# naver/dust3r

Hardware: NVIDIA H100
Metric: image-pairs/sec (512x384, ViT-L/B+DPT) (higher is better)
Workload: dtype bf16

## Files before the change

### dust3r_b200/csrc/attention_wgmma.cu

```cuda
#include "d3r_common.cuh"
#include "sm90_ptx.cuh"
#include "elementwise.h"
#include "prof.h"
#include "pdl.cuh"

namespace d3r {
namespace attn {

namespace wg {

constexpr int BQ = 128, BK = 128, D = 64;
constexpr int kThreads = 384;
constexpr int kTileBytes = 128 * 64 * 2;
constexpr int kPBytes = 2 * 64 * 128 * 2;
template <bool P_SMEM>
struct Smem {
  static constexpr int kP = P_SMEM ? 2 * kPBytes : 0;
  static constexpr int kBytes = kTileBytes  + 2 * kTileBytes  + 2 * kTileBytes  + kP + 128  + 1024;
  static_assert(kBytes <= 227 * 1024, "shared memory of one CTA");
};

template <bool P_SMEM>
__global__ void __launch_bounds__(kThreads, 1)
attention_kernel(const __grid_constant__ CUtensorMap tmap_q, const __grid_constant__ CUtensorMap tmap_k,
                 const __grid_constant__ CUtensorMap tmap_v, __nv_bfloat16* __restrict__ out, long long ldo, int Nq, int Nk,
                 int heads, int total_tiles, float scale_log2) {
  extern __shared__ uint8_t smem_raw[];
  uint8_t* smem = reinterpret_cast<uint8_t*>((reinterpret_cast<uintptr_t>(smem_raw) + 1023) & ~uintptr_t(1023));
  uint8_t* s_q = smem;
  uint8_t* s_k = s_q + kTileBytes;
  uint8_t* s_v = s_k + 2 * kTileBytes;
  uint8_t* s_p = s_v + 2 * kTileBytes;
  uint64_t* bars = reinterpret_cast<uint64_t*>(s_p + Smem<P_SMEM>::kP);
  uint64_t* q_full = bars + 0;
  uint64_t* q_empty = bars + 1;
  uint64_t* k_full = bars + 2;
  uint64_t* k_empty = bars + 4;
  uint64_t* v_full = bars + 6;
  uint64_t* v_empty = bars + 8;

  const int warp = threadIdx.x >> 5, lane = threadIdx.x & 31;
  const int nq_tiles = (Nq + BQ - 1) / BQ;
  const int nblk = (Nk + BK - 1) / BK;
  auto tile_coords = [&](int t, int& q0, int& h, int& b) {
    q0 = (t % nq_tiles) * BQ;
    h = (t / nq_tiles) % heads;
    b = t / (nq_tiles * heads);
  };

  if (threadIdx.x == 0) {
    ptx::prefetch_tmap(&tmap_q);
    ptx::prefetch_tmap(&tmap_k);
    ptx::prefetch_tmap(&tmap_v);
    ptx::mbar_init(ptx::smem_u32(q_full), 1);
    ptx::mbar_init(ptx::smem_u32(q_empty), 8);
    for (int s = 0; s < 2; ++s) {
      ptx::mbar_init(ptx::smem_u32(&k_full[s]), 1);
      ptx::mbar_init(ptx::smem_u32(&k_empty[s]), 8);
      ptx::mbar_init(ptx::smem_u32(&v_full[s]), 1);
      ptx::mbar_init(ptx::smem_u32(&v_empty[s]), 8);
    }
    ptx::fence_barrier_init();
  }
  __syncthreads();
  pdl::sync_with_predecessor();

  if (warp < 4) {
    ptx::setmaxnreg_dec<24>();
    if (warp == 0 && ptx::elect_one()) {
      uint32_t g = 0, it = 0;
      for (int t = blockIdx.x; t < total_tiles; t += gridDim.x, ++it) {
        int q0, h, b;
        tile_coords(t, q0, h, b);
        ptx::mbar_wait(ptx::smem_u32(q_empty), (it & 1) ^ 1);
        ptx::mbar_arrive_expect_tx(ptx::smem_u32(q_full), kTileBytes);
        ptx::tma_load_3d(ptx::smem_u32(s_q), &tmap_q, ptx::smem_u32(q_full), h * D, q0, b);
        for (int j = 0; j < nblk; ++j, ++g) {
          const int st = g & 1;
          const uint32_t ph = (g >> 1) & 1;
          ptx::mbar_wait(ptx::smem_u32(&k_empty[st]), ph ^ 1);
          ptx::mbar_arrive_expect_tx(ptx::smem_u32(&k_full[st]), kTileBytes);
          ptx::tma_load_3d(ptx::smem_u32(s_k + st * kTileBytes), &tmap_k, ptx::smem_u32(&k_full[st]), h * D, j * BK, b);
          ptx::mbar_wait(ptx::smem_u32(&v_empty[st]), ph ^ 1);
          ptx::mbar_arrive_expect_tx(ptx::smem_u32(&v_full[st]), kTileBytes);
          ptx::tma_load_3d(ptx::smem_u32(s_v + st * kTileBytes), &tmap_v, ptx::smem_u32(&v_full[st]), h * D, j * BK, b);
        }
      }
    }
  } else {
    ptx::setmaxnreg_inc<240>();
    const int cw = (threadIdx.x >> 7) - 1;
    const int wq = warp & 3, q = lane & 3;
    uint8_t* s_pw = s_p + cw * kPBytes;
    uint32_t g = 0, it = 0;
    for (int t = blockIdx.x; t < total_tiles; t += gridDim.x, ++it) {
      int q0, h, b;
      tile_coords(t, q0, h, b);
      float m_run[2] = {-INFINITY, -INFINITY}, l_run[2] = {0.f, 0.f};
      float o[32];
#pragma unroll
      for (int i = 0; i < 32; ++i) o[i] = 0.f;
      ptx::mbar_wait(ptx::smem_u32(q_full), it & 1);
      const uint64_t dq = ptx::desc_kmajor_sw128(ptx::smem_u32(s_q + cw * 64 * 128));
      for (int j = 0; j < nblk; ++j, ++g) {
        const int st = g & 1;
        const uint32_t ph = (g >> 1) & 1;
        float s[64];
        ptx::mbar_wait(ptx::smem_u32(&k_full[st]), ph);
        const uint64_t dk = ptx::desc_kmajor_sw128(ptx::smem_u32(s_k + st * kTileBytes));
        ptx::wgmma_fence();
#pragma unroll
        for (int k = 0; k < D / 16; ++k) ptx::wgmma_m64n128k16_ss(s, dq + uint64_t(2 * k), dk + uint64_t(2 * k), k ? 1u : 0u);
        ptx::wgmma_commit();
        ptx::wgmma_wait<0>();
        ptx::reg_fence(s);
        if (lane == 0) {
          ptx::mbar_arrive(ptx::smem_u32(&k_empty[st]));
          if (j == nblk - 1) ptx::mbar_arrive(ptx::smem_u32(q_empty));
        }
        const int nvalid = Nk - j * BK;
        if (nvalid < BK) {
#pragma unroll
          for (int n = 0; n < 16; ++n)
#pragma unroll
            for (int e = 0; e < 2; ++e)
              if (8 * n + 2 * q + e >= nvalid) { s[4 * n + e] = -INFINITY; s[4 * n + 2 + e] = -INFINITY; }
        }
        float ms[2];
#pragma unroll
        for (int hh = 0; hh < 2; ++hh) {
          float mx = -INFINITY;
#pragma unroll
          for (int n = 0; n < 16; ++n) mx = fmaxf(mx, fmaxf(s[4 * n + 2 * hh], s[4 * n + 2 * hh + 1]));
          mx = fmaxf(mx, __shfl_xor_sync(0xffffffffu, mx, 1));
          mx = fmaxf(mx, __shfl_xor_sync(0xffffffffu, mx, 2));
          const float m_new = fmaxf(m_run[hh], mx);
          const float corr = ptx::ex2_approx((m_run[hh] - m_new) * scale_log2);
          m_run[hh] = m_new;
          l_run[hh] *= corr;
#pragma unroll
          for (int n = 0; n < 8; ++n) { o[4 * n + 2 * hh] *= corr; o[4 * n + 2 * hh + 1] *= corr; }
          ms[hh] = m_new * scale_log2;
        }
        uint32_t pk[32];
#pragma unroll
        for (int n = 0; n < 16; ++n)
#pragma unroll
          for (int hh = 0; hh < 2; ++hh) {
            const float p0 = ptx::ex2_approx(fmaf(s[4 * n + 2 * hh], scale_log2, -ms[hh]));
            const float p1 = ptx::ex2_approx(fmaf(s[4 * n + 2 * hh + 1], scale_log2, -ms[hh]));
            l_run[hh] += p0 + p1;
            pk[2 * n + hh] = pack_bf16x2(p0, p1);
          }
        ptx::mbar_wait(ptx::smem_u32(&v_full[st]), ph);
        const uint32_t sv = ptx::smem_u32(s_v + st * kTileBytes);
        if constexpr (P_SMEM) {
#pragma unroll
          for (int n = 0; n < 16; ++n)
#pragma unroll
            for (int hh = 0; hh < 2; ++hh) {
              const int r = wq * 16 + (lane >> 2) + 8 * hh;
              *reinterpret_cast<uint32_t*>(s_pw + (n >> 3) * (64 * 128) + r * 128 + (((n & 7) ^ (r & 7)) << 4) + 4 * q) = pk[2 * n + hh];
            }
          ptx::fence_proxy_async();
          asm volatile("bar.sync %0, 128;" ::"r"(1 + cw) : "memory");
          const uint32_t sp = ptx::smem_u32(s_pw);
          ptx::wgmma_fence();
#pragma unroll
          for (int kk = 0; kk < BK / 16; ++kk)
            ptx::wgmma_m64n64k16_ss_tb(o, ptx::desc_kmajor_sw128(sp + (kk >> 2) * (64 * 128)) + uint64_t(2 * (kk & 3)),
                                       ptx::desc_mnmajor_sw128(sv + kk * 16 * 128), 1u);
        } else {
          ptx::wgmma_fence();
#pragma unroll
          for (int kk = 0; kk < BK / 16; ++kk) ptx::wgmma_m64n64k16_rs_tb(o, pk + 4 * kk, ptx::desc_mnmajor_sw128(sv + kk * 16 * 128), 1u);
        }
        ptx::wgmma_commit();
        ptx::wgmma_wait<0>();
        ptx::reg_fence(o);
        if constexpr (P_SMEM) asm volatile("bar.sync %0, 128;" ::"r"(1 + cw) : "memory");
        if (lane == 0) ptx::mbar_arrive(ptx::smem_u32(&v_empty[st]));
      }
#pragma unroll
      for (int hh = 0; hh < 2; ++hh) {
        float l = l_run[hh];
        l += __shfl_xor_sync(0xffffffffu, l, 1);
        l += __shfl_xor_sync(0xffffffffu, l, 2);
        const float inv = 1.f / l;
        const int qrow = q0 + cw * 64 + wq * 16 + (lane >> 2) + 8 * hh;
        if (qrow < Nq) {
          __nv_bfloat16* orow = out + ((long long)b * Nq + qrow) * ldo + h * D + 2 * q;
#pragma unroll
          for (int n = 0; n < 8; ++n)
            *reinterpret_cast<uint32_t*>(orow + 8 * n) = pack_bf16x2(o[4 * n + 2 * hh] * inv, o[4 * n + 2 * hh + 1] * inv);
        }
      }
    }
  }
}

}

template <bool P_SMEM>
static int launch_attention(const CUtensorMap& mq, const CUtensorMap& mk, const CUtensorMap& mv, void* out, long long ldo, int B, int heads,
                            int Nq, int Nk, float scale, cudaStream_t st) {
  static unsigned long long attr_devices = 0;
  if (first_launch_on_this_device(attr_devices))
    D3R_CUDA(cudaFuncSetAttribute(wg::attention_kernel<P_SMEM>, cudaFuncAttributeMaxDynamicSharedMemorySize, wg::Smem<P_SMEM>::kBytes));
  const int total_tiles = ((Nq + wg::BQ - 1) / wg::BQ) * heads * B;
  const int slots = num_sms();
  const int rounds = (total_tiles + slots - 1) / slots;
  const int grid = (total_tiles + rounds - 1) / rounds;
  prof::Scope scope(P_SMEM ? "attention_wgmma_psmem" : "attention_wgmma", st, 4.0 * double(B) * heads * double(Nq) * double(Nk) * 64.0);
  D3R_CUDA(pdl::launch(wg::attention_kernel<P_SMEM>, dim3(grid), dim3(wg::kThreads), size_t(wg::Smem<P_SMEM>::kBytes), st, mq, mk, mv,
                       (__nv_bfloat16*)out, ldo, Nq, Nk, heads, total_tiles, scale * 1.4426950408889634f));
  D3R_LAUNCH_CHECK();
  return D3R_OK;
}

static int make_map(CUtensorMap* m, const void* base, long long ld, int cols, int N, int B, int box_rows) {
  const cuuint64_t dims[3] = {(cuuint64_t)cols, (cuuint64_t)N, (cuuint64_t)B};
  const cuuint64_t str[2] = {(cuuint64_t)ld * 2, (cuuint64_t)N * ld * 2};
  const cuuint32_t box[3] = {64, (cuuint32_t)box_rows, 1};
  return encode_tensor_map(m, base, 3, dims, str, box, "attention");
}

static int g_impl = 3;

int attention_hd64(const void* q, long long ldq, const void* k, long long ldk, const void* v, long long ldv, void* out,
                   long long ldo, int B, int heads, int Nq, int Nk, float scale, cudaStream_t st) {
  D3R_CHECK_ARG(q && k && v && out && B > 0 && heads > 0 && Nq > 0 && Nk > 0, "attention: bad arguments");
  D3R_CHECK_ARG(ldq % 8 == 0 && ldk % 8 == 0 && ldv % 8 == 0 && ldo % 8 == 0, "attention: row strides must be multiples of 8");
  D3R_CHECK_ARG(((uintptr_t)q & 15) == 0 && ((uintptr_t)k & 15) == 0 && ((uintptr_t)v & 15) == 0 && ((uintptr_t)out & 15) == 0,
                "attention: pointers must be 16-byte aligned");
  CUtensorMap mq, mk, mv;
  int rc;
  if ((rc = make_map(&mq, q, ldq, heads * 64, Nq, B, wg::BQ))) return rc;
  if ((rc = make_map(&mk, k, ldk, heads * 64, Nk, B, wg::BK))) return rc;
  if ((rc = make_map(&mv, v, ldv, heads * 64, Nk, B, wg::BK))) return rc;
  if (g_impl == 2) return launch_attention<true>(mq, mk, mv, out, ldo, B, heads, Nq, Nk, scale, st);
  return launch_attention<false>(mq, mk, mv, out, ldo, B, heads, Nq, Nk, scale, st);
}

}
}

extern "C" void d3r_set_attention_impl(int32_t impl) { d3r::attn::g_impl = (impl == 2) ? 2 : 3; }

extern "C" int d3r_attention_hd64(const void* q, int64_t ldq, const void* k, int64_t ldk, const void* v, int64_t ldv, void* out,
                                  int64_t ldo, int32_t B, int32_t heads, int32_t Nq, int32_t Nk, float scale, void* stream) {
  return d3r::attn::attention_hd64(q, ldq, k, ldk, v, ldv, out, ldo, B, heads, Nq, Nk, scale, (cudaStream_t)stream);
}
```

Before: 234.3.

## Pipeline QK^T and PV WGMMAs across key blocks with three consumer warpgroups

```diff
diff --git a/dust3r_b200/csrc/attention_wgmma.cu b/dust3r_b200/csrc/attention_wgmma.cu
--- a/dust3r_b200/csrc/attention_wgmma.cu
+++ b/dust3r_b200/csrc/attention_wgmma.cu
@@ -9,56 +9,135 @@
 
 namespace wg {
 
-constexpr int BQ = 128, BK = 128, D = 64;
-constexpr int kThreads = 384;
+constexpr int BK = 128, D = 64;
 constexpr int kTileBytes = 128 * 64 * 2;
 constexpr int kPBytes = 2 * 64 * 128 * 2;
-template <bool P_SMEM>
-struct Smem {
-  static constexpr int kP = P_SMEM ? 2 * kPBytes : 0;
-  static constexpr int kBytes = kTileBytes  + 2 * kTileBytes  + 2 * kTileBytes  + kP + 128  + 1024;
-  static_assert(kBytes <= 227 * 1024, "shared memory of one CTA");
+constexpr int kSerialReg = 1, kSmemP = 2, kPipelined = 3;
+template <int IMPL>
+struct Cfg {
+  static constexpr bool kPSmem = IMPL == kSmemP;
+  static constexpr bool kPipe = IMPL == kPipelined;
+  static constexpr int kConsumers = kPipe ? 3 : 2;
+  static constexpr int BQ = 64 * kConsumers;
+  static constexpr int kThreads = 128 * (1 + kConsumers);
+  static constexpr int kConsumerRegs = kConsumers == 3 ? 160 : 240;
+  static_assert(128 * (24 + kConsumers * kConsumerRegs) <= 65536, "register file of one SM");
+  static constexpr int kStages = 2;
+  static constexpr int kP = kPSmem ? 2 * kPBytes : 0;
+  static constexpr int kSmemBytes =
+      BQ * 128  + kStages * kTileBytes  + kStages * kTileBytes  + kP + 128  + 1024;
+  static_assert(kSmemBytes <= 227 * 1024, "shared memory of one CTA");
+  static_assert(4 * kStages + 2 <= 16, "barriers fit their 128 bytes");
 };
 
-template <bool P_SMEM>
-__global__ void __launch_bounds__(kThreads, 1)
+
+__device__ __forceinline__ void mask_keys(float (&s)[64], int nvalid, int q) {
+  if (nvalid < BK) {
+#pragma unroll
+    for (int n = 0; n < 16; ++n)
+#pragma unroll
+      for (int e = 0; e < 2; ++e)
+        if (8 * n + 2 * q + e >= nvalid) { s[4 * n + e] = -INFINITY; s[4 * n + 2 + e] = -INFINITY; }
+  }
+}
+
+__device__ __forceinline__ void softmax_max(const float (&s)[64], float (&m_run)[2], float (&l_run)[2], float (&corr)[2],
+                                            float (&ms)[2], float scale_log2) {
+#pragma unroll
+  for (int hh = 0; hh < 2; ++hh) {
+    float mx = -INFINITY;
+#pragma unroll
+    for (int n = 0; n < 16; ++n) mx = fmaxf(mx, fmaxf(s[4 * n + 2 * hh], s[4 * n + 2 * hh + 1]));
+    mx = fmaxf(mx, __shfl_xor_sync(0xffffffffu, mx, 1));
+    mx = fmaxf(mx, __shfl_xor_sync(0xffffffffu, mx, 2));
+    const float m_new = fmaxf(m_run[hh], mx);
+    corr[hh] = ptx::ex2_approx((m_run[hh] - m_new) * scale_log2);
+    m_run[hh] = m_new;
+    l_run[hh] *= corr[hh];
+    ms[hh] = m_new * scale_log2;
+  }
+}
+
+__device__ __forceinline__ void rescale_o(float (&o)[32], const float (&corr)[2]) {
+#pragma unroll
+  for (int hh = 0; hh < 2; ++hh)
+#pragma unroll
+    for (int n = 0; n < 8; ++n) { o[4 * n + 2 * hh] *= corr[hh]; o[4 * n + 2 * hh + 1] *= corr[hh]; }
+}
+
+__device__ __forceinline__ void softmax_exp(float (&s)[64], const float (&ms)[2], float (&l_run)[2], float scale_log2) {
+#pragma unroll
+  for (int n = 0; n < 16; ++n)
+#pragma unroll
+    for (int hh = 0; hh < 2; ++hh) {
+      const float p0 = ptx::ex2_approx(fmaf(s[4 * n + 2 * hh], scale_log2, -ms[hh]));
+      const float p1 = ptx::ex2_approx(fmaf(s[4 * n + 2 * hh + 1], scale_log2, -ms[hh]));
+      l_run[hh] += p0 + p1;
+      s[4 * n + 2 * hh] = p0;
+      s[4 * n + 2 * hh + 1] = p1;
+    }
+}
+
+__device__ __forceinline__ void pack_p(const float (&p)[64], uint32_t (&pk)[32]) {
+#pragma unroll
+  for (int n = 0; n < 16; ++n)
+#pragma unroll
+    for (int hh = 0; hh < 2; ++hh) pk[2 * n + hh] = pack_bf16x2(p[4 * n + 2 * hh], p[4 * n + 2 * hh + 1]);
+}
+
+__device__ __forceinline__ void issue_s(float (&s)[64], uint64_t dq, uint64_t dk) {
+#pragma unroll
+  for (int k = 0; k < D / 16; ++k) ptx::wgmma_m64n128k16_ss(s, dq + uint64_t(2 * k), dk + uint64_t(2 * k), k ? 1u : 0u);
+}
+
+__device__ __forceinline__ void issue_pv_reg(float (&o)[32], const uint32_t (&pk)[32], uint32_t sv) {
+#pragma unroll
+  for (int kk = 0; kk < BK / 16; ++kk) ptx::wgmma_m64n64k16_rs_tb(o, pk + 4 * kk, ptx::desc_mnmajor_sw128(sv + kk * 16 * 128), 1u);
+}
+
+template <int IMPL>
+__global__ void __launch_bounds__(Cfg<IMPL>::kThreads, 1)
 attention_kernel(const __grid_constant__ CUtensorMap tmap_q, const __grid_constant__ CUtensorMap tmap_k,
                  const __grid_constant__ CUtensorMap tmap_v, __nv_bfloat16* __restrict__ out, long long ldo, int Nq, int Nk,
                  int heads, int total_tiles, float scale_log2) {
+  using C = Cfg<IMPL>;
+  constexpr int S = C::kStages;
   extern __shared__ uint8_t smem_raw[];
   uint8_t* smem = reinterpret_cast<uint8_t*>((reinterpret_cast<uintptr_t>(smem_raw) + 1023) & ~uintptr_t(1023));
   uint8_t* s_q = smem;
-  uint8_t* s_k = s_q + kTileBytes;
-  uint8_t* s_v = s_k + 2 * kTileBytes;
-  uint8_t* s_p = s_v + 2 * kTileBytes;
-  uint64_t* bars = reinterpret_cast<uint64_t*>(s_p + Smem<P_SMEM>::kP);
+  uint8_t* s_k = s_q + C::BQ * 128;
+  uint8_t* s_v = s_k + S * kTileBytes;
+  uint8_t* s_p = s_v + S * kTileBytes;
+  uint64_t* bars = reinterpret_cast<uint64_t*>(s_p + C::kP);
   uint64_t* q_full = bars + 0;
   uint64_t* q_empty = bars + 1;
   uint64_t* k_full = bars + 2;
-  uint64_t* k_empty = bars + 4;
-  uint64_t* v_full = bars + 6;
-  uint64_t* v_empty = bars + 8;
+  uint64_t* k_empty = bars + 2 + S;
+  uint64_t* v_full = bars + 2 + 2 * S;
+  uint64_t* v_empty = bars + 2 + 3 * S;
 
   const int warp = threadIdx.x >> 5, lane = threadIdx.x & 31;
-  const int nq_tiles = (Nq + BQ - 1) / BQ;
+  const int nq_tiles = (Nq + C::BQ - 1) / C::BQ;
   const int nblk = (Nk + BK - 1) / BK;
   auto tile_coords = [&](int t, int& q0, int& h, int& b) {
-    q0 = (t % nq_tiles) * BQ;
+    q0 = (t % nq_tiles) * C::BQ;
     h = (t / nq_tiles) % heads;
     b = t / (nq_tiles * heads);
   };
+  auto stage = [](uint32_t g) { return int(g % S); };
+  auto phase = [](uint32_t g) { return (g / S) & 1u; };
 
   if (threadIdx.x == 0) {
     ptx::prefetch_tmap(&tmap_q);
     ptx::prefetch_tmap(&tmap_k);
     ptx::prefetch_tmap(&tmap_v);
     ptx::mbar_init(ptx::smem_u32(q_full), 1);
-    ptx::mbar_init(ptx::smem_u32(q_empty), 8);
-    for (int s = 0; s < 2; ++s) {
+    ptx::mbar_init(ptx::smem_u32(q_empty), 4 * C::kConsumers);
+    for (int s = 0; s < S; ++s) {
       ptx::mbar_init(ptx::smem_u32(&k_full[s]), 1);
-      ptx::mbar_init(ptx::smem_u32(&k_empty[s]), 8);
+      ptx::mbar_init(ptx::smem_u32(&k_empty[s]), 4 * C::kConsumers);
       ptx::mbar_init(ptx::smem_u32(&v_full[s]), 1);
-      ptx::mbar_init(ptx::smem_u32(&v_empty[s]), 8);
+      ptx::mbar_init(ptx::smem_u32(&v_empty[s]), 4 * C::kConsumers);
     }
     ptx::fence_barrier_init();
   }
@@ -73,11 +152,11 @@
         int q0, h, b;
         tile_coords(t, q0, h, b);
         ptx::mbar_wait(ptx::smem_u32(q_empty), (it & 1) ^ 1);
-        ptx::mbar_arrive_expect_tx(ptx::smem_u32(q_full), kTileBytes);
+        ptx::mbar_arrive_expect_tx(ptx::smem_u32(q_full), C::BQ * 128);
         ptx::tma_load_3d(ptx::smem_u32(s_q), &tmap_q, ptx::smem_u32(q_full), h * D, q0, b);
         for (int j = 0; j < nblk; ++j, ++g) {
-          const int st = g & 1;
-          const uint32_t ph = (g >> 1) & 1;
+          const int st = stage(g);
+          const uint32_t ph = phase(g);
           ptx::mbar_wait(ptx::smem_u32(&k_empty[st]), ph ^ 1);
           ptx::mbar_arrive_expect_tx(ptx::smem_u32(&k_full[st]), kTileBytes);
           ptx::tma_load_3d(ptx::smem_u32(s_k + st * kTileBytes), &tmap_k, ptx::smem_u32(&k_full[st]), h * D, j * BK, b);
@@ -88,10 +167,15 @@
       }
     }
   } else {
-    ptx::setmaxnreg_inc<240>();
+    ptx::setmaxnreg_inc<C::kConsumerRegs>();
     const int cw = (threadIdx.x >> 7) - 1;
     const int wq = warp & 3, q = lane & 3;
     uint8_t* s_pw = s_p + cw * kPBytes;
+    auto k_smem = [&](uint32_t g) { return ptx::smem_u32(s_k + stage(g) * kTileBytes); };
+    auto v_smem = [&](uint32_t g) { return ptx::smem_u32(s_v + stage(g) * kTileBytes); };
+    auto release = [&](uint64_t* bar) {
+      if (lane == 0) ptx::mbar_arrive(ptx::smem_u32(bar));
+    };
     uint32_t g = 0, it = 0;
     for (int t = blockIdx.x; t < total_tiles; t += gridDim.x, ++it) {
       int q0, h, b;
@@ -102,84 +186,99 @@
       for (int i = 0; i < 32; ++i) o[i] = 0.f;
       ptx::mbar_wait(ptx::smem_u32(q_full), it & 1);
       const uint64_t dq = ptx::desc_kmajor_sw128(ptx::smem_u32(s_q + cw * 64 * 128));
-      for (int j = 0; j < nblk; ++j, ++g) {
-        const int st = g & 1;
-        const uint32_t ph = (g >> 1) & 1;
+      if constexpr (C::kPipe) {
         float s[64];
-        ptx::mbar_wait(ptx::smem_u32(&k_full[st]), ph);
-        const uint64_t dk = ptx::desc_kmajor_sw128(ptx::smem_u32(s_k + st * kTileBytes));
+        uint32_t pk[32];
+        float corr[2], ms[2];
+        ptx::mbar_wait(ptx::smem_u32(&k_full[stage(g)]), phase(g));
         ptx::wgmma_fence();
-#pragma unroll
-        for (int k = 0; k < D / 16; ++k) ptx::wgmma_m64n128k16_ss(s, dq + uint64_t(2 * k), dk + uint64_t(2 * k), k ? 1u : 0u);
+        issue_s(s, dq, ptx::desc_kmajor_sw128(k_smem(g)));
         ptx::wgmma_commit();
         ptx::wgmma_wait<0>();
         ptx::reg_fence(s);
-        if (lane == 0) {
-          ptx::mbar_arrive(ptx::smem_u32(&k_empty[st]));
-          if (j == nblk - 1) ptx::mbar_arrive(ptx::smem_u32(q_empty));
+        release(&k_empty[stage(g)]);
+        if (nblk == 1) release(q_empty);
+        mask_keys(s, Nk, q);
+        softmax_max(s, m_run, l_run, corr, ms, scale_log2);
+        softmax_exp(s, ms, l_run, scale_log2);
+        pack_p(s, pk);
+        ptx::mbar_wait(ptx::smem_u32(&v_full[stage(g)]), phase(g));
+        for (int j = 1; j < nblk; ++j) {
+          const uint32_t gc = g + j, gp = gc - 1;
+          ptx::mbar_wait(ptx::smem_u32(&k_full[stage(gc)]), phase(gc));
+          ptx::wgmma_fence();
+          issue_s(s, dq, ptx::desc_kmajor_sw128(k_smem(gc)));
+          ptx::wgmma_commit();
+          issue_pv_reg(o, pk, v_smem(gp));
+          ptx::wgmma_commit();
+          ptx::wgmma_wait<1>();
+          ptx::reg_fence(s);
+          release(&k_empty[stage(gc)]);
+          if (j == nblk - 1) release(q_empty);
+          mask_keys(s, Nk - j * BK, q);
+          softmax_max(s, m_run, l_run, corr, ms, scale_log2);
+          softmax_exp(s, ms, l_run, scale_log2);
+          ptx::mbar_wait(ptx::smem_u32(&v_full[stage(gc)]), phase(gc));
+          ptx::wgmma_wait<0>();
+          ptx::reg_fence(o);
+          release(&v_empty[stage(gp)]);
+          rescale_o(o, corr);
+          pack_p(s, pk);
         }
-        const int nvalid = Nk - j * BK;
-        if (nvalid < BK) {
-#pragma unroll
-          for (int n = 0; n < 16; ++n)
-#pragma unroll
-            for (int e = 0; e < 2; ++e)
-              if (8 * n + 2 * q + e >= nvalid) { s[4 * n + e] = -INFINITY; s[4 * n + 2 + e] = -INFINITY; }
-        }
-        float ms[2];
-#pragma unroll
-        for (int hh = 0; hh < 2; ++hh) {
-          float mx = -INFINITY;
-#pragma unroll
-          for (int n = 0; n < 16; ++n) mx = fmaxf(mx, fmaxf(s[4 * n + 2 * hh], s[4 * n + 2 * hh + 1]));
-          mx = fmaxf(mx, __shfl_xor_sync(0xffffffffu, mx, 1));
-          mx = fmaxf(mx, __shfl_xor_sync(0xffffffffu, mx, 2));
-          const float m_new = fmaxf(m_run[hh], mx);
-          const float corr = ptx::ex2_approx((m_run[hh] - m_new) * scale_log2);
-          m_run[hh] = m_new;
-          l_run[hh] *= corr;
-#pragma unroll
-          for (int n = 0; n < 8; ++n) { o[4 * n + 2 * hh] *= corr; o[4 * n + 2 * hh + 1] *= corr; }
-          ms[hh] = m_new * scale_log2;
-        }
-        uint32_t pk[32];
-#pragma unroll
-        for (int n = 0; n < 16; ++n)
-#pragma unroll
-          for (int hh = 0; hh < 2; ++hh) {
-            const float p0 = ptx::ex2_approx(fmaf(s[4 * n + 2 * hh], scale_log2, -ms[hh]));
-            const float p1 = ptx::ex2_approx(fmaf(s[4 * n + 2 * hh + 1], scale_log2, -ms[hh]));
-            l_run[hh] += p0 + p1;
-            pk[2 * n + hh] = pack_bf16x2(p0, p1);
-          }
-        ptx::mbar_wait(ptx::smem_u32(&v_full[st]), ph);
-        const uint32_t sv = ptx::smem_u32(s_v + st * kTileBytes);
-        if constexpr (P_SMEM) {
-#pragma unroll
-          for (int n = 0; n < 16; ++n)
-#pragma unroll
-            for (int hh = 0; hh < 2; ++hh) {
-              const int r = wq * 16 + (lane >> 2) + 8 * hh;
-              *reinterpret_cast<uint32_t*>(s_pw + (n >> 3) * (64 * 128) + r * 128 + (((n & 7) ^ (r & 7)) << 4) + 4 * q) = pk[2 * n + hh];
-            }
-          ptx::fence_proxy_async();
-          asm volatile("bar.sync %0, 128;" ::"r"(1 + cw) : "memory");
-          const uint32_t sp = ptx::smem_u32(s_pw);
-          ptx::wgmma_fence();
-#pragma unroll
-          for (int kk = 0; kk < BK / 16; ++kk)
-            ptx::wgmma_m64n64k16_ss_tb(o, ptx::desc_kmajor_sw128(sp + (kk >> 2) * (64 * 128)) + uint64_t(2 * (kk & 3)),
-                                       ptx::desc_mnmajor_sw128(sv + kk * 16 * 128), 1u);
-        } else {
-          ptx::wgmma_fence();
-#pragma unroll
-          for (int kk = 0; kk < BK / 16; ++kk) ptx::wgmma_m64n64k16_rs_tb(o, pk + 4 * kk, ptx::desc_mnmajor_sw128(sv + kk * 16 * 128), 1u);
-        }
+        const uint32_t gl = g + nblk - 1;
+        ptx::wgmma_fence();
+        issue_pv_reg(o, pk, v_smem(gl));
         ptx::wgmma_commit();
         ptx::wgmma_wait<0>();
         ptx::reg_fence(o);
-        if constexpr (P_SMEM) asm volatile("bar.sync %0, 128;" ::"r"(1 + cw) : "memory");
-        if (lane == 0) ptx::mbar_arrive(ptx::smem_u32(&v_empty[st]));
+        release(&v_empty[stage(gl)]);
+        g += nblk;
+      } else {
+        for (int j = 0; j < nblk; ++j, ++g) {
+          float s[64];
+          ptx::mbar_wait(ptx::smem_u32(&k_full[stage(g)]), phase(g));
+          ptx::wgmma_fence();
+          issue_s(s, dq, ptx::desc_kmajor_sw128(k_smem(g)));
+          ptx::wgmma_commit();
+          ptx::wgmma_wait<0>();
+          ptx::reg_fence(s);
+          release(&k_empty[stage(g)]);
+          if (j == nblk - 1) release(q_empty);
+          float corr[2], ms[2];
+          mask_keys(s, Nk - j * BK, q);
+          softmax_max(s, m_run, l_run, corr, ms, scale_log2);
+          rescale_o(o, corr);
+          softmax_exp(s, ms, l_run, scale_log2);
+          uint32_t pk[32];
+          pack_p(s, pk);
+          ptx::mbar_wait(ptx::smem_u32(&v_full[stage(g)]), phase(g));
+          const uint32_t sv = v_smem(g);
+          if constexpr (C::kPSmem) {
+#pragma unroll
+            for (int n = 0; n < 16; ++n)
+#pragma unroll
+              for (int hh = 0; hh < 2; ++hh) {
+                const int r = wq * 16 + (lane >> 2) + 8 * hh;
+                *reinterpret_cast<uint32_t*>(s_pw + (n >> 3) * (64 * 128) + r * 128 + (((n & 7) ^ (r & 7)) << 4) + 4 * q) = pk[2 * n + hh];
+              }
+            ptx::fence_proxy_async();
+            asm volatile("bar.sync %0, 128;" ::"r"(1 + cw) : "memory");
+            const uint32_t sp = ptx::smem_u32(s_pw);
+            ptx::wgmma_fence();
+#pragma unroll
+            for (int kk = 0; kk < BK / 16; ++kk)
+              ptx::wgmma_m64n64k16_ss_tb(o, ptx::desc_kmajor_sw128(sp + (kk >> 2) * (64 * 128)) + uint64_t(2 * (kk & 3)),
+                                         ptx::desc_mnmajor_sw128(sv + kk * 16 * 128), 1u);
+          } else {
+            ptx::wgmma_fence();
+            issue_pv_reg(o, pk, sv);
+          }
+          ptx::wgmma_commit();
+          ptx::wgmma_wait<0>();
+          ptx::reg_fence(o);
+          if constexpr (C::kPSmem) asm volatile("bar.sync %0, 128;" ::"r"(1 + cw) : "memory");
+          release(&v_empty[stage(g)]);
+        }
       }
 #pragma unroll
       for (int hh = 0; hh < 2; ++hh) {
@@ -201,23 +300,6 @@
 
 }
 
-template <bool P_SMEM>
-static int launch_attention(const CUtensorMap& mq, const CUtensorMap& mk, const CUtensorMap& mv, void* out, long long ldo, int B, int heads,
-                            int Nq, int Nk, float scale, cudaStream_t st) {
-  static unsigned long long attr_devices = 0;
-  if (first_launch_on_this_device(attr_devices))
-    D3R_CUDA(cudaFuncSetAttribute(wg::attention_kernel<P_SMEM>, cudaFuncAttributeMaxDynamicSharedMemorySize, wg::Smem<P_SMEM>::kBytes));
-  const int total_tiles = ((Nq + wg::BQ - 1) / wg::BQ) * heads * B;
-  const int slots = num_sms();
-  const int rounds = (total_tiles + slots - 1) / slots;
-  const int grid = (total_tiles + rounds - 1) / rounds;
-  prof::Scope scope(P_SMEM ? "attention_wgmma_psmem" : "attention_wgmma", st, 4.0 * double(B) * heads * double(Nq) * double(Nk) * 64.0);
-  D3R_CUDA(pdl::launch(wg::attention_kernel<P_SMEM>, dim3(grid), dim3(wg::kThreads), size_t(wg::Smem<P_SMEM>::kBytes), st, mq, mk, mv,
-                       (__nv_bfloat16*)out, ldo, Nq, Nk, heads, total_tiles, scale * 1.4426950408889634f));
-  D3R_LAUNCH_CHECK();
-  return D3R_OK;
-}
-
 static int make_map(CUtensorMap* m, const void* base, long long ld, int cols, int N, int B, int box_rows) {
   const cuuint64_t dims[3] = {(cuuint64_t)cols, (cuuint64_t)N, (cuuint64_t)B};
   const cuuint64_t str[2] = {(cuuint64_t)ld * 2, (cuuint64_t)N * ld * 2};
@@ -225,7 +307,28 @@
   return encode_tensor_map(m, base, 3, dims, str, box, "attention");
 }
 
-static int g_impl = 3;
+template <int IMPL>
+static int launch_attention(const void* q, long long ldq, const CUtensorMap& mk, const CUtensorMap& mv, void* out, long long ldo, int B,
+                            int heads, int Nq, int Nk, float scale, cudaStream_t st) {
+  using C = wg::Cfg<IMPL>;
+  CUtensorMap mq;
+  if (int rc = make_map(&mq, q, ldq, heads * 64, Nq, B, C::BQ)) return rc;
+  static unsigned long long attr_devices = 0;
+  if (first_launch_on_this_device(attr_devices))
+    D3R_CUDA(cudaFuncSetAttribute(wg::attention_kernel<IMPL>, cudaFuncAttributeMaxDynamicSharedMemorySize, C::kSmemBytes));
+  const int total_tiles = ((Nq + C::BQ - 1) / C::BQ) * heads * B;
+  const int slots = num_sms();
+  const int rounds = (total_tiles + slots - 1) / slots;
+  const int grid = (total_tiles + rounds - 1) / rounds;
+  const char* tag = IMPL == wg::kPipelined ? "attention_wgmma" : IMPL == wg::kSmemP ? "attention_wgmma_psmem" : "attention_wgmma_serial";
+  prof::Scope scope(tag, st, 4.0 * double(B) * heads * double(Nq) * double(Nk) * 64.0);
+  D3R_CUDA(pdl::launch(wg::attention_kernel<IMPL>, dim3(grid), dim3(C::kThreads), size_t(C::kSmemBytes), st, mq, mk, mv,
+                       (__nv_bfloat16*)out, ldo, Nq, Nk, heads, total_tiles, scale * 1.4426950408889634f));
+  D3R_LAUNCH_CHECK();
+  return D3R_OK;
+}
+
+static int g_impl = wg::kPipelined;
 
 int attention_hd64(const void* q, long long ldq, const void* k, long long ldk, const void* v, long long ldv, void* out,
                    long long ldo, int B, int heads, int Nq, int Nk, float scale, cudaStream_t st) {
@@ -233,19 +336,21 @@
   D3R_CHECK_ARG(ldq % 8 == 0 && ldk % 8 == 0 && ldv % 8 == 0 && ldo % 8 == 0, "attention: row strides must be multiples of 8");
   D3R_CHECK_ARG(((uintptr_t)q & 15) == 0 && ((uintptr_t)k & 15) == 0 && ((uintptr_t)v & 15) == 0 && ((uintptr_t)out & 15) == 0,
                 "attention: pointers must be 16-byte aligned");
-  CUtensorMap mq, mk, mv;
+  CUtensorMap mk, mv;
   int rc;
-  if ((rc = make_map(&mq, q, ldq, heads * 64, Nq, B, wg::BQ))) return rc;
   if ((rc = make_map(&mk, k, ldk, heads * 64, Nk, B, wg::BK))) return rc;
   if ((rc = make_map(&mv, v, ldv, heads * 64, Nk, B, wg::BK))) return rc;
-  if (g_impl == 2) return launch_attention<true>(mq, mk, mv, out, ldo, B, heads, Nq, Nk, scale, st);
-  return launch_attention<false>(mq, mk, mv, out, ldo, B, heads, Nq, Nk, scale, st);
-}
-
-}
-}
-
-extern "C" void d3r_set_attention_impl(int32_t impl) { d3r::attn::g_impl = (impl == 2) ? 2 : 3; }
+  if (g_impl == wg::kSmemP) return launch_attention<wg::kSmemP>(q, ldq, mk, mv, out, ldo, B, heads, Nq, Nk, scale, st);
+  if (g_impl == wg::kSerialReg) return launch_attention<wg::kSerialReg>(q, ldq, mk, mv, out, ldo, B, heads, Nq, Nk, scale, st);
+  return launch_attention<wg::kPipelined>(q, ldq, mk, mv, out, ldo, B, heads, Nq, Nk, scale, st);
+}
+
+}
+}
+
+extern "C" void d3r_set_attention_impl(int32_t impl) {
+  d3r::attn::g_impl = (impl == 1 || impl == 2) ? impl : d3r::attn::wg::kPipelined;
+}
 
 extern "C" int d3r_attention_hd64(const void* q, int64_t ldq, const void* k, int64_t ldk, const void* v, int64_t ldv, void* out,
                                   int64_t ldo, int32_t B, int32_t heads, int32_t Nq, int32_t Nk, float scale, void* stream) {
```

New measurement: 238.6, median of 6. 1.8% higher.
